# Intsights/PySubstringSearch

Measured on AMD Instinct MI355X. Metric: queries/sec (batched) + index-build GB/s on 512MB chunk, 1/2/4/8 GPU, higher is better.
Workload: dtype u64

## Files before the change

### pysubstringsearch_amd/csrc/msd_sort.hip

```cpp
#include "msd_sort.h"

#include <algorithm>
#include <vector>

#include "prims.h"
#include "scan.h"
#include "text_keys.h"

namespace pss {

constexpr int MSD_D = 10;
constexpr u32 MSD_BINS = 1u << MSD_D;
constexpr int MSD_BLOCK = 512;
constexpr int MSD_WAVES = MSD_BLOCK / kWave;
constexpr int MSD_IPT = 16;
constexpr u32 MSD_TILE = MSD_BLOCK * MSD_IPT;
constexpr u32 MSD_WIN = 6144;
#ifndef PSS_LS_WINDOW
#define PSS_LS_WINDOW 8
#endif
constexpr u32 MSD_TILE_CAP = 8184 - PSS_LS_WINDOW;
constexpr u32 MSD_MAX_BUCKET = 4088;
constexpr int MSD_TAG_BITS = MSD_D + 1;
constexpr u32 MSD_TAG_SPAN = 1u << MSD_TAG_BITS;
constexpr int MSD_RAW_TAG_BITS = 6;
constexpr u32 MSD_RAW_TAG_SPAN = 1u << MSD_RAW_TAG_BITS;
constexpr u32 MSD_G1_RANGES = 1024;
constexpr u32 MSD_G2_RANGE = 16 * MSD_TILE;

struct MsdRange {
    u32 seg, start, end;
};

struct MsdTile2 {
    u32 start, count, d_last;
};

struct MsdArgs {
    const u8 *codes;
    int code_bits, key_chars, plus_one, key_drop;
    u32 n;
    int key_bits;
    int idx_bits;
    u32 tiles_per_range1, num_ranges1;
    u32 *T;
    u32 *J1;
    u32 *J;
    MsdRange *ranges2;
    u32 *seg_first;
    u32 *counters;
    const u64 *dense;
    const u64 *in;
    u64 *out;
    int lsd;
    u32 *T2;
    const u32 *Jb;
    const struct MsdTile2 *tiles2;
    u32 *status;
    const u8 *raw;
    const u8 *lut;
    u8 *codes_out;
    u32 *bad;
};


template <bool FROM_TEXT>
__device__ __forceinline__ void msd_load_tile(const MsdArgs &a, u32 base, u32 valid, u64 (&elem)[MSD_IPT], u32 (&dig)[MSD_IPT],
                                              int shift2)
{
    const u32 tid = threadIdx.x;
    if (FROM_TEXT) {
        const u32 i0 = base + tid * MSD_IPT;
        u64 key[MSD_IPT] = {};
        if (i0 < a.n) text_keys16(a.codes, i0, a.code_bits, a.key_chars, a.plus_one, a.key_drop, a.n, key);
        const int rest_bits = a.key_bits - MSD_D;
        const u64 rest_mask = (1ull << rest_bits) - 1ull;
#pragma unroll
        for (int r = 0; r < MSD_IPT; ++r) {
            dig[r] = (u32)(key[r] >> rest_bits) & (MSD_BINS - 1u);
            elem[r] = ((key[r] & rest_mask) << a.idx_bits) | (u64)(i0 + r);
        }
    } else {
#pragma unroll
        for (int r = 0; r < MSD_IPT; ++r) {
            const u32 p = r * MSD_BLOCK + tid;
            elem[r] = p < valid ? a.in[base + p] : 0ull;
            dig[r] = (u32)(elem[r] >> shift2) & (MSD_BINS - 1u);
        }
    }
}

template <bool FROM_TEXT>
__device__ __forceinline__ bool msd_valid(u32 base, u32 valid, int r, u32 n)
{
    const u32 tid = threadIdx.x;
    (void)base;
    (void)n;
    return FROM_TEXT ? (tid * MSD_IPT + r < valid) : (r * MSD_BLOCK + tid < valid);
}

template <bool FROM_TEXT>
__global__ __launch_bounds__(MSD_BLOCK) void msd_hist_kernel(MsdArgs a)
{
    __shared__ u32 hist[MSD_BINS];
    __shared__ u32 histb[FROM_TEXT ? MSD_BINS : 1];
    const u32 tid = threadIdx.x, r = blockIdx.x;
    u32 e0, e1;
    if (FROM_TEXT) {
        if (r >= a.num_ranges1) return;
        e0 = r * a.tiles_per_range1 * MSD_TILE;
        const u64 end = (u64)(r + 1) * a.tiles_per_range1 * MSD_TILE;
        e1 = end < a.n ? (u32)end : a.n;
    } else {
        if (r >= a.counters[0]) return;
        e0 = a.ranges2[r].start;
        e1 = a.ranges2[r].end;
    }
    for (u32 i = tid; i < MSD_BINS; i += MSD_BLOCK) {
        hist[i] = 0;
        if (FROM_TEXT) histb[i] = 0;
    }
    __syncthreads();
    const int shift2 = a.idx_bits + a.key_bits - 2 * MSD_D;
    if (FROM_TEXT) {
        const int b = a.code_bits;
        const int top = a.lsd ? 2 * MSD_D : MSD_D;
        const int m = (top + b - 1) / b;
        const u32 wmask = (m * b >= 32) ? ~0u : ((1u << (m * b)) - 1u);
        const int down = m * b - top;
        uint4 nlo = make_uint4(0, 0, 0, 0), nhi = nlo;
        if (e0 + tid * MSD_IPT < e1) {
            const uint4 *p = reinterpret_cast<const uint4 *>(a.codes + e0 + tid * MSD_IPT);
            nlo = p[0];
            nhi = p[1];
        }
        for (u32 base = e0; base < e1; base += MSD_TILE) {
            const u32 i0 = base + tid * MSD_IPT;
            const uint4 lo = nlo, hi = nhi;
            if ((u64)i0 + MSD_TILE < e1) {
                const uint4 *p = reinterpret_cast<const uint4 *>(a.codes + i0 + MSD_TILE);
                nlo = p[0];
                nhi = p[1];
            }
            if (i0 >= e1) continue;
            const u64 q[4] = {(u64)lo.x | ((u64)lo.y << 32), (u64)lo.z | ((u64)lo.w << 32),
                              (u64)hi.x | ((u64)hi.y << 32), (u64)hi.z | ((u64)hi.w << 32)};
            auto sym = [&](u32 j) -> u32 { return (u32)(q[j >> 3] >> ((j & 7u) * 8u)) & 0xffu; };
            u32 win = 0;
            for (int t = 0; t < m; ++t) win = (win << b) | sym((u32)t);
#pragma unroll
            for (int r = 0; r < MSD_IPT; ++r) {
                if (r > 0) win = ((win << b) | sym((u32)(m - 1 + r))) & wmask;
                if (i0 + r < e1) {
                    const u32 tp = win >> down;
                    atomicAdd(&hist[tp & (MSD_BINS - 1u)], 1u);
// ... 789 lines not shown
                const u64 at = (u64)sfx[j] + f.h0;
                if (at < f.n) key[j] = text_key_at(f.codes, (u32)at, f.code_bits, f.key_syms, f.plus_one, f.n);
            }
        }
        bool same = false;
#pragma unroll
        for (int j = 0; j < FIN_MAX; ++j) {
#pragma unroll
            for (int l = j + 1; l < FIN_MAX; ++l) {
                if ((u32)l < g) {
                    same |= key[j] == key[l];
                    rk[l] += key[j] < key[l] ? 1u : 0u;
                    rk[j] += key[j] < key[l] ? 0u : 1u;
                }
            }
        }
        if (same) continue;
        settled = true;
#pragma unroll
        for (int j = 0; j < FIN_MAX; ++j) {
            if ((u32)j < g) {
                sa_out[ps + rk[j]] = sfx[j];
                atomicOr(&done[(q + j) >> 5], 1u << ((q + j) & 31u));
            }
        }
    }
    __builtin_amdgcn_fence(__ATOMIC_ACQ_REL, "wavefront");
    __builtin_amdgcn_wave_barrier();
    if (__ballot(settled) == 0) return;
    u32 kept = 0;
    for (u32 base = 0; base < c; base += kWave) {
        const u32 i = base + lane;
        u32 ps = 0, v = 0;
        bool keep = false;
        if (i < c) {
            record(i, ps, v);
            const u32 q = ps - e0;
            keep = ((done[q >> 5] >> (q & 31u)) & 1u) == 0;
        }
        const u64 km = __ballot(keep);
        __builtin_amdgcn_fence(__ATOMIC_ACQ_REL, "wavefront");
        __builtin_amdgcn_wave_barrier();
        if (keep) {
            const u32 o = e0 + kept + mbcnt(km);
            st_pos[o] = ps;
            st_idx[o] = v;
        }
        kept += (u32)__popcll(km);
    }
    if (lane == 0) blk_cnt[t] = kept | ((c - kept) << 16);
}


__global__ __launch_bounds__(MSD_BLOCK) void msd_local_sort_kernel(const u64 *in, const MsdTile *tiles, int rem_bits, int idx_bits,
                                                                     u32 *sa_out, const u32 *tile_list, int fused, MsdEmit em_val)
{
    const MsdEmit *em = fused ? &em_val : nullptr;
    __shared__ __attribute__((aligned(16))) u64 exch[MSD_TILE];
    __shared__ u32 wave_hist[MSD_WAVES][256];
    __shared__ u32 scr[MSD_WAVES + 1];
    const u32 tid = threadIdx.x, lane = tid & 63u, wave = tid >> 6;
    const u32 t = tile_list ? tile_list[blockIdx.x] : blockIdx.x;
    const MsdTile td = tiles[t];
    const u32 e0 = td.e0, count = td.count;
    for (u32 i = tid; i < MSD_WAVES * 256; i += MSD_BLOCK) (&wave_hist[0][0])[i] = 0;
    __syncthreads();
    int seg_bits = 0;
    while ((1u << seg_bits) < td.nb) ++seg_bits;
    const u64 tag_base = (u64)td.tag0 << (rem_bits + idx_bits);
    u64 key[MSD_IPT];
#pragma unroll
    for (int r = 0; r < MSD_IPT; ++r) {
        const u32 p = wave * (kWave * MSD_IPT) + r * kWave + lane;
        key[r] = p < count ? in[e0 + p] - tag_base : ~0ull;
    }
    const int sort_bits = rem_bits + seg_bits;
    for (int shift = idx_bits; shift < idx_bits + sort_bits; shift += 8) {
        const int left = idx_bits + sort_bits - shift;
        const u32 dmask = left >= 8 ? 0xffu : ((1u << left) - 1u);
        u32 rank[MSD_IPT], prev[MSD_IPT];
#pragma unroll
        for (int r = 0; r < MSD_IPT; ++r) {
            const bool pad = wave * (kWave * MSD_IPT) + r * kWave + lane >= count;
            const u32 d = pad ? dmask : ((u32)(key[r] >> shift) & dmask);
            const u64 peers = match_digit8(d, ~0ull);
            const u32 below = mbcnt(peers);
            prev[r] = 0;
            if (below == 0) prev[r] = atomicAdd(&wave_hist[wave][d], (u32)__popcll(peers));
            rank[r] = below | ((u32)__builtin_ctzll(peers) << 16);
        }
#pragma unroll
        for (int r = 0; r < MSD_IPT; ++r) rank[r] = __shfl(prev[r], (int)(rank[r] >> 16)) + (rank[r] & 0xffffu);
        __syncthreads();
        {
            u32 c[MSD_WAVES];
            u32 total = 0;
            if (tid < 256) {
#pragma unroll
                for (int w = 0; w < MSD_WAVES; ++w) {
                    c[w] = wave_hist[w][tid];
                    total += c[w];
                }
            }
            const u32 incl = wave_incl_sum(total);
            if (lane == kWave - 1) scr[wave] = incl;
            __syncthreads();
            if (tid < 256) {
                u32 run = incl - total;
                for (u32 w = 0; w < wave; ++w) run += scr[w];
#pragma unroll
                for (int w = 0; w < MSD_WAVES; ++w) {
                    wave_hist[w][tid] = run;
                    run += c[w];
                }
            }
        }
        __syncthreads();
#pragma unroll
        for (int r = 0; r < MSD_IPT; ++r) {
            const bool pad = wave * (kWave * MSD_IPT) + r * kWave + lane >= count;
            const u32 d = pad ? dmask : ((u32)(key[r] >> shift) & dmask);
            exch[wave_hist[wave][d] + rank[r]] = key[r];
        }
        __syncthreads();
        for (u32 i = tid; i < MSD_WAVES * 256; i += MSD_BLOCK) (&wave_hist[0][0])[i] = 0;
#pragma unroll
        for (int r = 0; r < MSD_IPT; ++r) key[r] = exch[wave * (kWave * MSD_IPT) + r * kWave + lane];
        __syncthreads();
    }
    if (sort_bits <= 0) {
#pragma unroll
        for (int r = 0; r < MSD_IPT; ++r) exch[wave * (kWave * MSD_IPT) + r * kWave + lane] = key[r];
        __syncthreads();
    }
    if (tid == 0) scr[0] = 0;
    __syncthreads();
    msd_emit_tile(exch, count, e0, idx_bits, sa_out, em, &scr[0]);
    __syncthreads();
    if (em && tid == 0) em->blk_cnt[t] = scr[0];
}


#ifndef PSS_LS_BIN_BITS
#define PSS_LS_BIN_BITS 12
#endif
constexpr int LS_BIN_BITS = PSS_LS_BIN_BITS;
constexpr u32 LS_BINS = 1u << LS_BIN_BITS;
constexpr u32 LS_WORDS = LS_BINS / 2;
constexpr u32 LS_KMAX = 64;
#ifndef PSS_LS_GROUP
#define PSS_LS_GROUP 1
#endif
constexpr int LS_GROUP = PSS_LS_GROUP;
constexpr int LS_WINDOW = PSS_LS_WINDOW;

__global__ __launch_bounds__(256) void msd_tile_desc_kernel(const u32 *cstart, const u32 *tile_first, u32 nt, u32 ne, u32 n,
                                                              MsdTile *tiles, const u32 *cj, const u64 *ntp, const u64 *nep)
{
    const u32 t = blockIdx.x * blockDim.x + threadIdx.x;
    if (ntp) {
        nt = (u32)*ntp;
        ne = (u32)*nep;
    }
    if (t >= nt) return;
    const u32 k0 = tile_first[t], k1 = tile_first[t + 1];
    const u32 e0 = cstart[k0], e1 = k1 < ne ? cstart[k1] : n;
    if (cj) {
        const u32 t0 = cj[k0] & (MSD_RAW_TAG_SPAN - 1u), t1 = cj[k1 - 1] & (MSD_RAW_TAG_SPAN - 1u);
        tiles[t] = MsdTile{e0, e1 - e0, t0, t1 - t0 + 1u};
    } else {
        tiles[t] = MsdTile{e0, e1 - e0, k0 & (MSD_TAG_SPAN - 1u), k1 - k0};
    }
}

__device__ __forceinline__ void keep_load(u64 &v) { asm volatile("" : "+v"(v)); }

__device__ __forceinline__ void lds_barrier()
{
    asm volatile("s_waitcnt lgkmcnt(0)\n\ts_barrier" ::: "memory");
}

__global__ __launch_bounds__(MSD_BLOCK, 4) void msd_local_fast_kernel(const u64 *in, const MsdTile *tiles, u32 nt, int rem_bits,
                                                                     int idx_bits, u32 *sa_out, u32 *fail_list, u32 *fail_count,
                                                                     int fused, MsdEmit em_val, const u64 *nt_dev,
                                                                     const u32 *counters_dev, const u32 *bad_dev)
{
    if (nt_dev) {
        if (counters_dev[1] > MSD_MAX_BUCKET || (bad_dev && *bad_dev)) return;
        nt = (u32)*nt_dev;
    }
    const MsdEmit *em = fused ? &em_val : nullptr;
    __shared__ __attribute__((aligned(16))) u64 lds_all[MSD_TILE + LS_WORDS];
    u64 *const exch = lds_all;
    u32 *const hist = reinterpret_cast<u32 *>(lds_all + MSD_TILE);
    u32 *const hist2 = hist + LS_WORDS;
    u32 *const scr = reinterpret_cast<u32 *>(&exch[MSD_TILE - 8]);
    u32 &s_fail = scr[MSD_WAVES + 2];
    const u32 tid = threadIdx.x;
    const u32 stride = gridDim.x;
    u32 t = blockIdx.x;
    if (t >= nt) return;
    MsdTile cur = tiles[t];
    MsdTile nxt = t + stride < nt ? tiles[t + stride] : MsdTile{0, 0, 0, 0};
    u64 pe[MSD_IPT];
    auto prefetch = [&](const MsdTile &d) {
#pragma unroll
        for (int r = 0; r < MSD_IPT; ++r) {
            const u32 p = r * MSD_BLOCK + tid;
            pe[r] = p < d.count ? in[d.e0 + p] : 0ull;
        }
    };
    prefetch(cur);
    for (u32 i = tid; i < LS_WORDS; i += MSD_BLOCK) hist[i] = 0;
    if (tid == 0) {
        s_fail = 0;
        scr[MSD_WAVES + 3] = 0;
    }
    lds_barrier();
    u32 prev_t = 0;
    bool prev_ok = false;
    for (;;) {
        const u32 count = cur.count, e0 = cur.e0;
        const u32 rows = (count + MSD_BLOCK - 1) / MSD_BLOCK;
        int seg_bits = 0;
        while ((1u << seg_bits) < cur.nb) ++seg_bits;
        const u64 tag_base = (u64)cur.tag0 << (rem_bits + idx_bits);
        const int sort_bits = rem_bits + seg_bits;
        const int bin_shift = idx_bits + (sort_bits > LS_BIN_BITS ? sort_bits - LS_BIN_BITS : 0);
        u64 e[MSD_IPT];
#pragma unroll
        for (int r = 0; r < MSD_IPT; ++r) {
            e[r] = ~0ull;
            if ((u32)r < rows) {
                const u32 p = r * MSD_BLOCK + tid;
                if (p < count) {
                    e[r] = pe[r] - tag_base;
                    const u32 bin = (u32)(e[r] >> bin_shift);
                    atomicAdd(&hist[bin >> 1], 1u << (16u * (bin & 1u)));
                }
            }
        }
        const bool more = t + stride < nt;
        if (more) prefetch(nxt);
        lds_barrier();
        if (tid == 0) {
            if (em && prev_ok) em->blk_cnt[prev_t] = scr[MSD_WAVES + 3];
            s_fail = 0;
            scr[MSD_WAVES + 3] = 0;
        }
        {
            constexpr int LS_WPT = LS_WORDS / MSD_BLOCK;
            static_assert(LS_WPT * MSD_BLOCK == (int)LS_WORDS && LS_WPT >= 1, "bins split evenly over the threads");
            u32 c[2 * LS_WPT];
            u32 sum = 0;
#pragma unroll
            for (int j = 0; j < LS_WPT; ++j) {
                const u32 wv = hist[LS_WPT * tid + j];
                c[2 * j] = wv & 0xffffu;
                c[2 * j + 1] = wv >> 16;
                sum += c[2 * j] + c[2 * j + 1];
            }
            const u32 incl = wave_incl_sum(sum);
            if (lane_id() == kWave - 1) scr[wave_id()] = incl;
            lds_barrier();
            u32 ex = incl - sum;
            for (int w = 0; w < wave_id(); ++w) ex += scr[w];
#pragma unroll
            for (int j = 0; j < LS_WPT; ++j) {
                const u32 lo = ex, hi = ex + c[2 * j];
                hist[LS_WPT * tid + j] = hist2[LS_WPT * tid + j] = lo | (hi << 16);
                ex = hi + c[2 * j + 1];
            }
        }
        lds_barrier();
#pragma unroll
        for (int r = 0; r < MSD_IPT; ++r) {
            if ((u32)r < rows) {
                const u32 p = r * MSD_BLOCK + tid;
                if (p < count) {
                    const u32 bin = (u32)(e[r] >> bin_shift), sh = 16u * (bin & 1u);
                    exch[(atomicAdd(&hist2[bin >> 1], 1u << sh) >> sh) & 0xffffu] = e[r];
                }
            }
        }
        if (tid < (u32)LS_WINDOW) exch[count + tid] = ~0ull;
        lds_barrier();
        const u16 *const starts16 = reinterpret_cast<const u16 *>(hist);
        u32 rk[MSD_IPT];
#pragma unroll
        for (int g = 0; g < MSD_IPT; g += LS_GROUP) {
            if ((u32)g < rows) {
                u64 x[LS_GROUP];
                u32 s0[LS_GROUP], sm[LS_GROUP];
#pragma unroll
                for (int j = 0; j < LS_GROUP; ++j) x[j] = exch[(g + j) * MSD_BLOCK + tid];
#pragma unroll
                for (int j = 0; j < LS_GROUP; ++j) {
                    const u32 bin = (u32)(x[j] >> bin_shift) & (LS_BINS - 1u);
                    s0[j] = starts16[bin];
                }
                u64 y[LS_GROUP][LS_WINDOW];
#pragma unroll
                for (int j = 0; j < LS_GROUP; ++j) {
#pragma unroll
                    for (int k = 0; k < LS_WINDOW; ++k) y[j][k] = exch[s0[j] + k];
                }
#pragma unroll
                for (int j = 0; j < LS_GROUP; ++j) {
                    u32 c = 0;
#pragma unroll
                    for (int k = 0; k < LS_WINDOW; ++k) {
                        keep_load(y[j][k]);
                        c += y[j][k] < x[j] ? 1u : 0u;
                    }
                    sm[j] = c;
                }
#pragma unroll
                for (int j = 0; j < LS_GROUP; ++j) {
                    const u32 p = (g + j) * MSD_BLOCK + tid;
                    if (p < count && ((y[j][LS_WINDOW - 1] ^ x[j]) >> bin_shift) == 0) {
                        const u32 bin = (u32)(x[j] >> bin_shift) & (LS_BINS - 1u);
                        const u32 s1 = bin + 1u < LS_BINS ? (u32)starts16[min(bin + 1u, LS_BINS - 1u)] : count;
                        const u32 len = s1 - s0[j];
                        if (len > LS_KMAX) {
                            s_fail = 1;
                        } else {
                            for (u32 q = s0[j] + LS_WINDOW; q < s0[j] + len; ++q) sm[j] += exch[q] < x[j] ? 1u : 0u;
                        }
                    }
                    e[g + j] = x[j];
                    rk[g + j] = s0[j] + sm[j];
                }
            } else {
#pragma unroll
                for (int j = 0; j < LS_GROUP; ++j) rk[g + j] = 0;
            }
        }
        lds_barrier();
        const bool failed = s_fail != 0;
        if (failed) {
            if (tid == 0) fail_list[atomicAdd(fail_count, 1u)] = t;
        } else {
#pragma unroll
            for (int r = 0; r < MSD_IPT; ++r) {
                if ((u32)r < rows) {
                    const u32 p = r * MSD_BLOCK + tid;
                    if (p < count) exch[rk[r]] = e[r];
                }
            }
        }
        for (u32 i = tid; i < LS_WORDS; i += MSD_BLOCK) hist[i] = 0;
        lds_barrier();
        if (!failed) {
            const u32 imask = (u32)((1ull << idx_bits) - 1ull);
            u32 *const s_count = &scr[MSD_WAVES + 3];
#pragma unroll
            for (int g = 0; g < MSD_IPT; g += LS_GROUP) {
                if ((u32)g < rows) {
                    u64 cur[LS_GROUP], prv[LS_GROUP], nxt[LS_GROUP];
#pragma unroll
                    for (int j = 0; j < LS_GROUP; ++j) {
                        const u32 p = (g + j) * MSD_BLOCK + tid;
                        cur[j] = exch[p];
                        prv[j] = exch[p ? p - 1 : 0];
                        nxt[j] = exch[p + 1];
                    }
#pragma unroll
                    for (int j = 0; j < LS_GROUP; ++j) {
                        keep_load(cur[j]);
                        keep_load(prv[j]);
                        keep_load(nxt[j]);
                    }
#pragma unroll
                    for (int j = 0; j < LS_GROUP; ++j) {
                        const u32 p = (g + j) * MSD_BLOCK + tid;
                        if (p < count) {
                            const u64 kx = cur[j] >> idx_bits;
                            const bool tie = p > 0 && (prv[j] >> idx_bits) == kx;
                            const u32 sfx = (u32)cur[j] & imask;
                            sa_out[e0 + p] = sfx | ((tie && em == nullptr) ? 0x80000000u : 0u);
                            if (em != nullptr) {
                                const bool tie_next = p + 1 < count && (nxt[j] >> idx_bits) == kx;
                                if (tie || tie_next) {
                                    const u32 slot = e0 + atomicAdd(s_count, 1u);
                                    em->st_pos[slot] = e0 + p;
                                    em->st_idx[slot] = sfx | (tie ? 0x80000000u : 0u);
                                }
                            }
                        }
                    }
                }
            }
        }
        prev_t = t;
        prev_ok = !failed;
        if (!more) break;
        t += stride;
        cur = nxt;
        nxt = t + stride < nt ? tiles[t + stride] : MsdTile{0, 0, 0, 0};
    }
    if (em) {
        lds_barrier();
        if (tid == 0 && prev_ok) em->blk_cnt[prev_t] = scr[MSD_WAVES + 3];
    }
}

#include "ss_sort_impl.h"


static size_t msd_max_tiles(uint32_t n)
{
    return (size_t)n / (SS_WIN / 2) + ((size_t)MSD_BINS * MSD_BINS) / MSD_RAW_TAG_SPAN + 8;
}

static size_t msd_max_tiles2(uint32_t n) { return (size_t)n / MSD_TILE2 + MSD_BINS + 8; }

static bool msd_use_lsd(uint32_t n)
{
    const char *e = knob("PSS_MSD_LSD");
    return !(e && atoi(e) == 0) && n < (1u << 30);
}

size_t msd_workspace_bytes(uint32_t n)
{
    const size_t max_ranges2 = (size_t)n / MSD_G2_RANGE + MSD_BINS + 8;
    const size_t nbk = (size_t)MSD_BINS * MSD_BINS;
    return max_ranges2 * MSD_BINS * 4
           + (MSD_BINS + 8) * 4
           + (nbk + 8) * 4
           + max_ranges2 * sizeof(MsdRange) + (MSD_BINS + 8) * 4 + 64
           + (nbk + 8) * 8
           + (nbk + 8) * 4
           + (msd_max_tiles(n) + 32) * 8
           + (msd_max_tiles(n) + 32) * 16
           + (msd_max_tiles(n) + 32) * sizeof(MsdTile)
           + (SC_MAX_BLOCKS + 8) * 8 + 8192
           + (size_t)MSD_BINS * MSD_G1_RANGES * 4 + (MSD_BINS + 8) * 4
           + msd_max_tiles2(n) * (sizeof(MsdTile2) + (size_t)MSD_BINS * 4)
           + (nbk + 8) * 4 + 4096;
}

int msd_max_key_bits(uint32_t n)
{
    int ib = 1;
    while ((1ull << ib) < (u64)n) ++ib;
    const int after2 = 64 + MSD_D - (msd_use_lsd(n) ? MSD_RAW_TAG_BITS : MSD_TAG_BITS) - ib + MSD_D;
    return std::min(after2, 64 + MSD_D - ib);
}

int msd_suffix_sort(DeviceCtx *ctx, const TextKeys *text, uint32_t n, int key_bits, uint64_t *A[2], uint32_t *sa_out,
                    void *work, uint32_t *h_small, bool profile, MsdStats *stats, bool *accepted, MsdActive *active,
                    const MsdFront *front)
{
    *accepted = false;
    hipStream_t s = ctx->stream;
    int ib = 1;
    while ((1ull << ib) < (u64)n) ++ib;
    if (key_bits < 2 * MSD_D + 1 || key_bits > msd_max_key_bits(n) || n < 2) {
        set_error("msd_suffix_sort: key of %d bits does not fit (n = %u)", key_bits, n);
        return PSS_EINVAL;
    }
    const size_t max_ranges2 = (size_t)n / MSD_G2_RANGE + MSD_BINS + 8;
    const size_t nbk = (size_t)MSD_BINS * MSD_BINS;
    u8 *w = static_cast<u8 *>(work);
    size_t o = 0;
    auto carve = [&](size_t bytes) { u8 *p = w + o; o = round_up(o + bytes, 256); return p; };
    u32 *T = reinterpret_cast<u32 *>(carve(max_ranges2 * MSD_BINS * 4));
    u32 *J1 = reinterpret_cast<u32 *>(carve((MSD_BINS + 8) * 4));
    u32 *J = reinterpret_cast<u32 *>(carve((nbk + 8) * 4));
    MsdRange *ranges2 = reinterpret_cast<MsdRange *>(carve(max_ranges2 * sizeof(MsdRange)));
    u32 *seg_first = reinterpret_cast<u32 *>(carve((MSD_BINS + 8) * 4));
    u32 *counters = reinterpret_cast<u32 *>(carve(64));
    u64 *ranks = reinterpret_cast<u64 *>(carve((nbk + 8) * 8));
    u32 *cstart = reinterpret_cast<u32 *>(carve((nbk + 8) * 4));
    const size_t max_tiles = msd_max_tiles(n);
    MsdTile *tiles_all = reinterpret_cast<MsdTile *>(carve((max_tiles + 16) * sizeof(MsdTile)));
    u32 *tile_first = reinterpret_cast<u32 *>(carve((max_tiles + 16) * 8));
    u32 *blk_cnt = reinterpret_cast<u32 *>(carve((max_tiles + 8) * 4));
    u64 *dst_off = reinterpret_cast<u64 *>(carve((max_tiles + 8) * 8));
    u64 *partial = reinterpret_cast<u64 *>(carve((SC_MAX_BLOCKS + 8) * 8));
    u64 *d_total = partial + SC_MAX_BLOCKS;
    const bool lsd = msd_use_lsd(n);
    const size_t max_tiles2 = msd_max_tiles2(n);
    u32 *T2 = nullptr, *Jb = nullptr, *status = nullptr, *cj = nullptr;
    MsdTile2 *tiles2 = nullptr;
    if (lsd) {
        T2 = reinterpret_cast<u32 *>(carve((size_t)MSD_BINS * MSD_G1_RANGES * 4));
        Jb = reinterpret_cast<u32 *>(carve((MSD_BINS + 8) * 4));
        tiles2 = reinterpret_cast<MsdTile2 *>(carve(max_tiles2 * sizeof(MsdTile2)));
        status = reinterpret_cast<u32 *>(carve(max_tiles2 * MSD_BINS * 4));
        cj = reinterpret_cast<u32 *>(carve((nbk + 8) * 4));
    }

    MsdArgs a;
    memset(&a, 0, sizeof a);
    a.codes = text->codes;
    a.code_bits = text->code_bits;
    a.key_chars = text->key_chars;
    a.plus_one = text->plus_one;
    a.key_drop = text->drop;
    a.n = n;
    a.key_bits = key_bits;
    a.idx_bits = ib;
    const u32 num_tiles = (u32)(((u64)n + MSD_TILE - 1) / MSD_TILE);
    a.tiles_per_range1 = (num_tiles + MSD_G1_RANGES - 1) / MSD_G1_RANGES;
    a.num_ranges1 = (num_tiles + a.tiles_per_range1 - 1) / a.tiles_per_range1;
    a.T = T;
    a.J1 = J1;
    a.J = J;
    a.ranges2 = ranges2;
    a.seg_first = seg_first;
    a.counters = counters;
    a.lsd = lsd ? 1 : 0;
    a.T2 = T2;
    a.Jb = Jb;
    a.tiles2 = tiles2;
    a.status = status;

    hipEvent_t ev[8] = {};
    int nev = 0;
    struct EvGuard {
        hipEvent_t *e;
        int *n;
        ~EvGuard()
        {
            for (int i = 0; i < *n; ++i) (void)hipEventDestroy(e[i]);
        }
    } guard{ev, &nev};
    auto mark = [&]() -> int {
        if (profile && nev < 8) {
            PSS_HIP(hipEventCreate(&ev[nev]));
            PSS_HIP(hipEventRecord(ev[nev], s));
            ++nev;
        }
        return PSS_OK;
    };

    PSS_HIP(hipMemsetAsync(counters, 0, 64, s));
    a.out = A[0];
    if (front) {
        a.raw = front->raw;
        a.lut = front->lut;
        a.codes_out = const_cast<u8 *>(text->codes);
// ... 440 lines not shown
```

### pysubstringsearch_amd/csrc/prims.h

```cpp
#pragma once
#include <hip/hip_runtime.h>

#include <cstdint>

namespace pss {

typedef uint8_t u8;
typedef uint16_t u16;
typedef uint32_t u32;
typedef uint64_t u64;

constexpr int kWave = 64;

__device__ __forceinline__ int lane_id() { return threadIdx.x & (kWave - 1); }
__device__ __forceinline__ int wave_id() { return threadIdx.x >> 6; }

__device__ __forceinline__ u32 mbcnt(u64 mask)
{
    return __builtin_amdgcn_mbcnt_hi((u32)(mask >> 32), __builtin_amdgcn_mbcnt_lo((u32)mask, 0u));
}

__device__ __forceinline__ u64 match_digit8(u32 d, u64 valid_mask)
{
    u64 peers = valid_mask;
#pragma unroll
    for (int s = 0; s < 8; s += 2) {
        const bool b0 = (d >> s) & 1u;
        const bool b1 = (d >> (s + 1)) & 1u;
        const u64 m0 = __ballot(b0);
        const u64 m1 = __ballot(b1);
        peers &= (b0 ? m0 : ~m0) & (b1 ? m1 : ~m1);
    }
    return peers;
}

__device__ __forceinline__ u32 wave_incl_sum(u32 v)
{
    const int lane = lane_id();
#pragma unroll
    for (int o = 1; o < kWave; o <<= 1) {
        u32 t = __shfl_up(v, o);
        if (lane >= o) v += t;
    }
    return v;
}
__device__ __forceinline__ u64 wave_incl_sum64(u64 v)
{
    const int lane = lane_id();
#pragma unroll
    for (int o = 1; o < kWave; o <<= 1) {
        u64 t = __shfl_up(v, o);
        if (lane >= o) v += t;
    }
    return v;
}
__device__ __forceinline__ u32 wave_incl_max(u32 v)
{
    const int lane = lane_id();
#pragma unroll
    for (int o = 1; o < kWave; o <<= 1) {
        u32 t = __shfl_up(v, o);
        if (lane >= o) v = max(v, t);
    }
    return v;
}

template <int WAVES>
__device__ __forceinline__ u32 block_excl_sum(u32 v, u32 *scratch, u32 *total)
{
    const u32 incl = wave_incl_sum(v);
    if (lane_id() == kWave - 1) scratch[wave_id()] = incl;
    __syncthreads();
    u32 base = 0, tot = 0;
#pragma unroll
    for (int w = 0; w < WAVES; ++w) {
        const u32 s = scratch[w];
        if (w < wave_id()) base += s;
        tot += s;
    }
    __syncthreads();
    if (total) *total = tot;
    return base + incl - v;
}

__device__ __forceinline__ u32 xcd_range_of_block(u32 b, u32 num_blocks)
{
    const u32 per = num_blocks >> 3;
    return (b & 7u) * per + (b >> 3);
}

__device__ __forceinline__ u64 load_u64_unaligned(const u8 *p)
{
    const uintptr_t a = (uintptr_t)p;
    const u32 *q = (const u32 *)(a & ~(uintptr_t)3);
    const u32 sh = (u32)(a & 3) * 8;
    const u32 w0 = q[0], w1 = q[1];
    if (sh == 0) return (u64)w0 | ((u64)w1 << 32);
    const u32 w2 = q[2];
    const u32 lo = (w0 >> sh) | (w1 << (32 - sh));
    const u32 hi = (w1 >> sh) | (w2 << (32 - sh));
    return (u64)lo | ((u64)hi << 32);
}

}
```

Before: 67.84.

## Specialize full/partial rows in local sort kernel and use DPP wave scan

Adds an ls_rows helper that keeps the row count in a scalar register and splits full rows, which need no bounds check, from the last partial row, then applies it to prefetch, histogram, scatter and emit loops. Replaces the shuffle-based wave prefix sum with a DPP row_shr/row_bcast scan and reads per-wave totals with two vector LDS loads. The tie-emission atomics move out of the main loop into a bitmask-driven pass, and the next-tile prefetch is issued unconditionally. The aim is to cut VALU branch and exec-mask overhead and shuffle latency; the costs are more code size and register pressure, and correctness depends on the DPP scan and the tie bitmask logic matching the old behaviour.

```diff
diff --git a/pysubstringsearch_amd/csrc/msd_sort.hip b/pysubstringsearch_amd/csrc/msd_sort.hip
--- a/pysubstringsearch_amd/csrc/msd_sort.hip
+++ b/pysubstringsearch_amd/csrc/msd_sort.hip
@@ -1,6 +1,7 @@
 #include "msd_sort.h"
 
 #include <algorithm>
+#include <type_traits>
 #include <vector>
 
 #include "prims.h"
@@ -1096,6 +1097,10 @@
 #define PSS_LS_GROUP 1
 #endif
 constexpr int LS_GROUP = PSS_LS_GROUP;
+#ifndef PSS_LS_SLOT_GROUP
+#define PSS_LS_SLOT_GROUP 1
+#endif
+constexpr int LS_SLOT_GROUP = PSS_LS_SLOT_GROUP;
 constexpr int LS_WINDOW = PSS_LS_WINDOW;
 
 __global__ __launch_bounds__(256) void msd_tile_desc_kernel(const u32 *cstart, const u32 *tile_first, u32 nt, u32 ne, u32 n,
@@ -1124,6 +1129,25 @@
     asm volatile("s_waitcnt lgkmcnt(0)\n\ts_barrier" ::: "memory");
 }
 
+template <int G, class F>
+__device__ __forceinline__ void ls_rows(u32 rows, F &&f)
+{
+    static_assert(MSD_IPT % G == 0, "the groups tile the rows");
+    rows = (u32)__builtin_amdgcn_readfirstlane((int)rows);
+    asm volatile("" : "+s"(rows));
+#pragma unroll
+    for (int g = 0; g < MSD_IPT; g += G) {
+        if ((u32)(g + G) < rows) {
+            f(std::true_type{}, g);
+            asm volatile("");
+        }
+        if (rows - 1u - (u32)g < (u32)G) {
+            asm volatile("");
+            f(std::false_type{}, g);
+        }
+    }
+}
+
 __global__ __launch_bounds__(MSD_BLOCK, 4) void msd_local_fast_kernel(const u64 *in, const MsdTile *tiles, u32 nt, int rem_bits,
                                                                      int idx_bits, u32 *sa_out, u32 *fail_list, u32 *fail_count,
                                                                      int fused, MsdEmit em_val, const u64 *nt_dev,
@@ -1140,7 +1164,7 @@
     u32 *const hist2 = hist + LS_WORDS;
     u32 *const scr = reinterpret_cast<u32 *>(&exch[MSD_TILE - 8]);
     u32 &s_fail = scr[MSD_WAVES + 2];
-    const u32 tid = threadIdx.x;
+    u32 tid = threadIdx.x;
     const u32 stride = gridDim.x;
     u32 t = blockIdx.x;
     if (t >= nt) return;
@@ -1148,11 +1172,11 @@
     MsdTile nxt = t + stride < nt ? tiles[t + stride] : MsdTile{0, 0, 0, 0};
     u64 pe[MSD_IPT];
     auto prefetch = [&](const MsdTile &d) {
-#pragma unroll
-        for (int r = 0; r < MSD_IPT; ++r) {
+        const u64 *const src = in + d.e0;
+        ls_rows<1>((d.count + MSD_BLOCK - 1) / MSD_BLOCK, [&](auto full, int r) __attribute__((always_inline)) {
             const u32 p = r * MSD_BLOCK + tid;
-            pe[r] = p < d.count ? in[d.e0 + p] : 0ull;
-        }
+            if (decltype(full)::value || p < d.count) pe[r] = src[p];
+        });
     };
     prefetch(cur);
     for (u32 i = tid; i < LS_WORDS; i += MSD_BLOCK) hist[i] = 0;
@@ -1171,21 +1195,18 @@
         const u64 tag_base = (u64)cur.tag0 << (rem_bits + idx_bits);
         const int sort_bits = rem_bits + seg_bits;
         const int bin_shift = idx_bits + (sort_bits > LS_BIN_BITS ? sort_bits - LS_BIN_BITS : 0);
+        asm volatile("" : "+v"(tid));
+        const u32 wave_no = (u32)__builtin_amdgcn_readfirstlane((int)(tid >> 6));
         u64 e[MSD_IPT];
-#pragma unroll
-        for (int r = 0; r < MSD_IPT; ++r) {
-            e[r] = ~0ull;
-            if ((u32)r < rows) {
-                const u32 p = r * MSD_BLOCK + tid;
-                if (p < count) {
-                    e[r] = pe[r] - tag_base;
-                    const u32 bin = (u32)(e[r] >> bin_shift);
-                    atomicAdd(&hist[bin >> 1], 1u << (16u * (bin & 1u)));
-                }
-            }
-        }
+        ls_rows<1>(rows, [&](auto full, int r) __attribute__((always_inline)) {
+            if (decltype(full)::value || r * MSD_BLOCK + tid < count) {
+                e[r] = pe[r] - tag_base;
+                const u32 bin = (u32)(e[r] >> bin_shift);
+                atomicAdd(&hist[bin >> 1], 1u << (16u * (bin & 1u)));
+            }
+        });
         const bool more = t + stride < nt;
-        if (more) prefetch(nxt);
+        prefetch(nxt);
         lds_barrier();
         if (tid == 0) {
             if (em && prev_ok) em->blk_cnt[prev_t] = scr[MSD_WAVES + 3];
@@ -1204,11 +1225,15 @@
                 c[2 * j + 1] = wv >> 16;
                 sum += c[2 * j] + c[2 * j + 1];
             }
-            const u32 incl = wave_incl_sum(sum);
-            if (lane_id() == kWave - 1) scr[wave_id()] = incl;
+            const u32 incl = wave_incl_sum_dpp(sum);
+            if ((tid & (kWave - 1u)) == kWave - 1u) scr[wave_no] = incl;
             lds_barrier();
+            static_assert(MSD_WAVES == 8, "two 16-byte reads hold the totals of all waves");
+            const uint4 w03 = *reinterpret_cast<const uint4 *>(&scr[0]), w47 = *reinterpret_cast<const uint4 *>(&scr[4]);
+            const u32 wtot[MSD_WAVES] = {w03.x, w03.y, w03.z, w03.w, w47.x, w47.y, w47.z, w47.w};
             u32 ex = incl - sum;
-            for (int w = 0; w < wave_id(); ++w) ex += scr[w];
+#pragma unroll
+            for (u32 w = 0; w + 1 < (u32)MSD_WAVES; ++w) ex += w < wave_no ? wtot[w] : 0u;
 #pragma unroll
             for (int j = 0; j < LS_WPT; ++j) {
                 const u32 lo = ex, hi = ex + c[2 * j];
@@ -1217,23 +1242,30 @@
             }
         }
         lds_barrier();
-#pragma unroll
-        for (int r = 0; r < MSD_IPT; ++r) {
-            if ((u32)r < rows) {
-                const u32 p = r * MSD_BLOCK + tid;
-                if (p < count) {
-                    const u32 bin = (u32)(e[r] >> bin_shift), sh = 16u * (bin & 1u);
-                    exch[(atomicAdd(&hist2[bin >> 1], 1u << sh) >> sh) & 0xffffu] = e[r];
+        ls_rows<LS_SLOT_GROUP>(rows, [&](auto full, int g) __attribute__((always_inline)) {
+            u32 slot[LS_SLOT_GROUP], sh[LS_SLOT_GROUP];
+#pragma unroll
+            for (int j = 0; j < LS_SLOT_GROUP; ++j) {
+                if (decltype(full)::value || (g + j) * MSD_BLOCK + tid < count) {
+                    const u32 bin = (u32)(e[g + j] >> bin_shift);
+                    sh[j] = 16u * (bin & 1u);
+                    slot[j] = atomicAdd(&hist2[bin >> 1], 1u << sh[j]);
                 }
             }
-        }
+#pragma unroll
+            for (int j = 0; j < LS_SLOT_GROUP; ++j) {
+                if (decltype(full)::value || (g + j) * MSD_BLOCK + tid < count) exch[(slot[j] >> sh[j]) & 0xffffu] = e[g + j];
+            }
+        });
         if (tid < (u32)LS_WINDOW) exch[count + tid] = ~0ull;
         lds_barrier();
         const u16 *const starts16 = reinterpret_cast<const u16 *>(hist);
         u32 rk[MSD_IPT];
+        u32 rank_rows = (u32)__builtin_amdgcn_readfirstlane((int)rows);
+        asm volatile("" : "+s"(rank_rows));
 #pragma unroll
         for (int g = 0; g < MSD_IPT; g += LS_GROUP) {
-            if ((u32)g < rows) {
+            if ((u32)g < rank_rows) {
                 u64 x[LS_GROUP];
                 u32 s0[LS_GROUP], sm[LS_GROUP];
 #pragma unroll
@@ -1261,8 +1293,7 @@
                 }
 #pragma unroll
                 for (int j = 0; j < LS_GROUP; ++j) {
-                    const u32 p = (g + j) * MSD_BLOCK + tid;
-                    if (p < count && ((y[j][LS_WINDOW - 1] ^ x[j]) >> bin_shift) == 0) {
+                    if (((y[j][LS_WINDOW - 1] ^ x[j]) >> bin_shift) == 0 && (g + j) * MSD_BLOCK + tid < count) {
                         const u32 bin = (u32)(x[j] >> bin_shift) & (LS_BINS - 1u);
                         const u32 s1 = bin + 1u < LS_BINS ? (u32)starts16[min(bin + 1u, LS_BINS - 1u)] : count;
                         const u32 len = s1 - s0[j];
@@ -1275,9 +1306,6 @@
                     e[g + j] = x[j];
                     rk[g + j] = s0[j] + sm[j];
                 }
-            } else {
-#pragma unroll
-                for (int j = 0; j < LS_GROUP; ++j) rk[g + j] = 0;
             }
         }
         lds_barrier();
@@ -1285,54 +1313,54 @@
         if (failed) {
             if (tid == 0) fail_list[atomicAdd(fail_count, 1u)] = t;
         } else {
-#pragma unroll
-            for (int r = 0; r < MSD_IPT; ++r) {
-                if ((u32)r < rows) {
-                    const u32 p = r * MSD_BLOCK + tid;
-                    if (p < count) exch[rk[r]] = e[r];
-                }
-            }
+            ls_rows<1>(rows, [&](auto full, int r) __attribute__((always_inline)) {
+                if (decltype(full)::value || r * MSD_BLOCK + tid < count) exch[rk[r]] = e[r];
+            });
         }
         for (u32 i = tid; i < LS_WORDS; i += MSD_BLOCK) hist[i] = 0;
         lds_barrier();
         if (!failed) {
             const u32 imask = (u32)((1ull << idx_bits) - 1ull);
-            u32 *const s_count = &scr[MSD_WAVES + 3];
-#pragma unroll
-            for (int g = 0; g < MSD_IPT; g += LS_GROUP) {
-                if ((u32)g < rows) {
-                    u64 cur[LS_GROUP], prv[LS_GROUP], nxt[LS_GROUP];
-#pragma unroll
-                    for (int j = 0; j < LS_GROUP; ++j) {
-                        const u32 p = (g + j) * MSD_BLOCK + tid;
-                        cur[j] = exch[p];
-                        prv[j] = exch[p ? p - 1 : 0];
-                        nxt[j] = exch[p + 1];
+            const u32 flag = em == nullptr ? 0x80000000u : 0u;
+            const u64 same = 1ull << idx_bits;
+            const u64 *const my = exch + tid;
+            u32 *const out = sa_out + e0 + tid;
+            u32 ties = 0;
+            ls_rows<LS_GROUP>(rows, [&](auto full, int g) __attribute__((always_inline)) {
+                u64 cur[LS_GROUP], prv[LS_GROUP], nxt[LS_GROUP];
+#pragma unroll
+                for (int j = 0; j < LS_GROUP; ++j) {
+                    const int o = (g + j) * MSD_BLOCK;
+                    cur[j] = my[o];
+                    prv[j] = o == 0 ? exch[tid - (tid != 0 ? 1u : 0u)] : my[o - 1];
+                    nxt[j] = my[o + 1];
+                }
+#pragma unroll
+                for (int j = 0; j < LS_GROUP; ++j) {
+                    keep_load(cur[j]);
+                    keep_load(prv[j]);
+                    keep_load(nxt[j]);
+                }
+#pragma unroll
+                for (int j = 0; j < LS_GROUP; ++j) {
+                    const int o = (g + j) * MSD_BLOCK;
+                    bool tie = (prv[j] ^ cur[j]) < same;
+                    if (o == 0) tie = tie && tid != 0;
+                    const bool tie_next = (nxt[j] ^ cur[j]) < same && (decltype(full)::value || o + tid + 1u < count);
+                    if (decltype(full)::value || o + tid < count) {
+                        out[o] = ((u32)cur[j] & imask) | (tie ? flag : 0u);
+                        ties |= ((tie || tie_next) ? 1u << (g + j) : 0u) | (tie ? 0x10000u << (g + j) : 0u);
                     }
-#pragma unroll
-                    for (int j = 0; j < LS_GROUP; ++j) {
-                        keep_load(cur[j]);
-                        keep_load(prv[j]);
-                        keep_load(nxt[j]);
-                    }
-#pragma unroll
-                    for (int j = 0; j < LS_GROUP; ++j) {
-                        const u32 p = (g + j) * MSD_BLOCK + tid;
-                        if (p < count) {
-                            const u64 kx = cur[j] >> idx_bits;
-                            const bool tie = p > 0 && (prv[j] >> idx_bits) == kx;
-                            const u32 sfx = (u32)cur[j] & imask;
-                            sa_out[e0 + p] = sfx | ((tie && em == nullptr) ? 0x80000000u : 0u);
-                            if (em != nullptr) {
-                                const bool tie_next = p + 1 < count && (nxt[j] >> idx_bits) == kx;
-                                if (tie || tie_next) {
-                                    const u32 slot = e0 + atomicAdd(s_count, 1u);
-                                    em->st_pos[slot] = e0 + p;
-                                    em->st_idx[slot] = sfx | (tie ? 0x80000000u : 0u);
-                                }
-                            }
-                        }
-                    }
+                }
+            });
+            if (em != nullptr) {
+                u32 *const s_count = &scr[MSD_WAVES + 3];
+                for (u32 m = ties & 0xffffu; m != 0; m &= m - 1u) {
+                    const u32 r = (u32)__builtin_ctz(m);
+                    const u32 p = r * MSD_BLOCK + tid;
+                    const u32 slot = e0 + atomicAdd(s_count, 1u);
+                    em->st_pos[slot] = e0 + p;
+                    em->st_idx[slot] = ((u32)exch[p] & imask) | ((ties >> (16u + r)) << 31);
                 }
             }
         }
diff --git a/pysubstringsearch_amd/csrc/prims.h b/pysubstringsearch_amd/csrc/prims.h
--- a/pysubstringsearch_amd/csrc/prims.h
+++ b/pysubstringsearch_amd/csrc/prims.h
@@ -42,6 +42,16 @@
         u32 t = __shfl_up(v, o);
         if (lane >= o) v += t;
     }
+    return v;
+}
+__device__ __forceinline__ u32 wave_incl_sum_dpp(u32 v)
+{
+    v += (u32)__builtin_amdgcn_update_dpp(0, (int)v, 0x111, 0xf, 0xf, false);
+    v += (u32)__builtin_amdgcn_update_dpp(0, (int)v, 0x112, 0xf, 0xf, false);
+    v += (u32)__builtin_amdgcn_update_dpp(0, (int)v, 0x114, 0xf, 0xf, false);
+    v += (u32)__builtin_amdgcn_update_dpp(0, (int)v, 0x118, 0xf, 0xf, false);
+    v += (u32)__builtin_amdgcn_update_dpp(0, (int)v, 0x142, 0xa, 0xf, false);
+    v += (u32)__builtin_amdgcn_update_dpp(0, (int)v, 0x143, 0xc, 0xf, false);
     return v;
 }
 __device__ __forceinline__ u64 wave_incl_sum64(u64 v)
```

New measurement: 71.33 (median of 6 runs). 1.05x the previous value.
